# Aedelon/ProteinBERT-PyTorch-Replication

Measured on AMD Instinct MI355X. Metric: sequences/sec (whole node) ProteinBERT pretrain L=512 at 1/2/4/8 MI355X, higher is better.
Workload: dtype bf16; 1 GPU; global_batch=2048, per_gpu_batch=2048, seq_len=512, parallelism=dp1, impl=hip, hip_graph=False

## Files before the change

### proteinbert_pytorch_replication_amd/ops/csrc/common.h

```cpp
#pragma once
#include <hip/hip_runtime.h>
#include <stdint.h>

#define PBX_EXPORT extern "C" __attribute__((visibility("default")))

typedef __attribute__((ext_vector_type(8))) short bf16x8_t;
typedef __attribute__((ext_vector_type(4))) short bf16x4_t;
typedef __attribute__((ext_vector_type(4))) float f32x4_t;
typedef __attribute__((ext_vector_type(16))) float f32x16_t;

__device__ __forceinline__ float bf2f(unsigned short h) {
  return __uint_as_float(((unsigned int)h) << 16);
}
__device__ __forceinline__ unsigned short f2bf(float f) {
  return __builtin_bit_cast(unsigned short, (__bf16)f);
}

__device__ __forceinline__ void gelu_parts(float x, float& cdf, float& pdf) {
  const float z = fabsf(x) * 0.70710678118654752f;
  const float t = __builtin_amdgcn_rcpf(fmaf(0.3275911f, z, 1.0f));
  const float e = __expf(-z * z);
  const float poly =
      t * fmaf(t, fmaf(t, fmaf(t, fmaf(t, 1.061405429f, -1.453152027f), 1.421413741f), -0.284496736f), 0.254829592f);
  const float erfz = fmaf(-poly, e, 1.0f);
  cdf = fmaf(0.5f, copysignf(erfz, x), 0.5f);
  pdf = 0.3989422804014327f * e;
}
__device__ __forceinline__ float gelu_f(float x) {
  float c, p;
  gelu_parts(x, c, p);
  return x * c;
}
__device__ __forceinline__ float gelu_grad_f(float x) {
  float c, p;
  gelu_parts(x, c, p);
  return fmaf(x, p, c);
}

typedef float f32x2 __attribute__((ext_vector_type(2)));

#ifndef PBX_GELU_EXACT
#define PBX_GELU_EXACT 0
#endif

template <int N, int MODE>
__device__ __forceinline__ void gelu_scalar_n(const f32x2* x, f32x2* g, f32x2* gd) {
  constexpr int M = 2 * N;
  float xs[M], t[M], e[M], pl[M];
#pragma unroll
  for (int i = 0; i < M; ++i) {
    xs[i] = (i & 1) ? x[i >> 1].y : x[i >> 1].x;
    t[i] = fmaf(fabsf(xs[i]), 0.23164190f, 1.0f);
    e[i] = MODE == 0 ? (xs[i] * -0.72134752044448170f) * xs[i]
                     : fmaf(xs[i] * xs[i], -0.72134752044448170f, -1.3257480647361592f);
  }
#pragma unroll
  for (int i = 0; i < M; ++i) {
    t[i] = __builtin_amdgcn_rcpf(t[i]);
    e[i] = __builtin_amdgcn_exp2f(e[i]);
  }
  constexpr float c5 = MODE == 0 ? -0.5307027145f : -1.3302744295891233f;
  constexpr float c4 = MODE == 0 ? 0.7265760135f : 1.8212559791077754f;
  constexpr float c3 = MODE == 0 ? -0.7107068705f : -1.7814779365698128f;
  constexpr float c2 = MODE == 0 ? 0.142248368f : 0.3565637812489156f;
  constexpr float c1 = MODE == 0 ? -0.127414796f : -0.31938153025994087f;
#pragma unroll
  for (int i = 0; i < M; ++i) pl[i] = fmaf(t[i], c5, c4);
#pragma unroll
  for (int i = 0; i < M; ++i) pl[i] = fmaf(t[i], pl[i], c3);
#pragma unroll
  for (int i = 0; i < M; ++i) pl[i] = fmaf(t[i], pl[i], c2);
#pragma unroll
  for (int i = 0; i < M; ++i) pl[i] = fmaf(t[i], pl[i], c1);
#pragma unroll
  for (int i = 0; i < M; ++i) pl[i] = fmaf(pl[i] * t[i], e[i], 0.5f);
#pragma unroll
  for (int i = 0; i < M; ++i) {
    float gv = 0.f, dv = 0.f;
    if (MODE == 0) {
      gv = fmaf(fabsf(xs[i]), pl[i], xs[i] * 0.5f);
    } else {
      const float Phi = copysignf(pl[i], xs[i]) + 0.5f;
      if (MODE == 2) gv = xs[i] * Phi;
      dv = fmaf(xs[i], e[i], Phi);
    }
    if (i & 1) {
      if (MODE != 1) g[i >> 1].y = gv;
      if (MODE != 0) gd[i >> 1].y = dv;
    } else {
      if (MODE != 1) g[i >> 1].x = gv;
      if (MODE != 0) gd[i >> 1].x = dv;
    }
  }
}

template <int N, int MODE>
__device__ __forceinline__ void gelu_logistic_n(const f32x2* x, f32x2* g, f32x2* gd) {
  constexpr int M = 2 * N;
  float xs[M], t[M], s[M];
#pragma unroll
  for (int i = 0; i < M; ++i) {
    xs[i] = (i & 1) ? x[i >> 1].y : x[i >> 1].x;
    t[i] = xs[i] * xs[i];
    s[i] = fmaf(t[i], -0.10053117f, -2.3073633f) * xs[i];
  }
#pragma unroll
  for (int i = 0; i < M; ++i) s[i] = __builtin_amdgcn_rcpf(__builtin_amdgcn_exp2f(s[i]) + 1.0f);
#pragma unroll
  for (int i = 0; i < M; ++i) {
    float gv = 0.f, dv = 0.f;
    if (MODE != 1) gv = xs[i] * s[i];
    if (MODE != 0) {
      const float kd = fmaf(t[i], 0.20904868f, 1.59934236f);
      dv = fmaf(xs[i] * fmaf(-s[i], s[i], s[i]), kd, s[i]);
    }
    if (i & 1) {
      if (MODE != 1) g[i >> 1].y = gv;
      if (MODE != 0) gd[i >> 1].y = dv;
    } else {
      if (MODE != 1) g[i >> 1].x = gv;
      if (MODE != 0) gd[i >> 1].x = dv;
    }
  }
}

template <int N, int MODE>
__device__ __forceinline__ void gelu_n(const f32x2* x, f32x2* g, f32x2* gd) {
  if constexpr (PBX_GELU_EXACT) gelu_scalar_n<N, MODE>(x, g, gd);
  else gelu_logistic_n<N, MODE>(x, g, gd);
}
template <int N, bool GRAD>
__device__ __forceinline__ void gelu2_fast_n(const f32x2* x, f32x2* out) {
  if (GRAD) gelu_n<N, 1>(x, nullptr, out);
  else gelu_n<N, 0>(x, out, nullptr);
}
template <int N>
__device__ __forceinline__ void gelu2_both_n(const f32x2* x, f32x2* g, f32x2* gd) {
  gelu_n<N, 2>(x, g, gd);
}

__device__ __forceinline__ float wave_reduce_sum(float v) {
#pragma unroll
  for (int o = 32; o > 0; o >>= 1) v += __shfl_xor(v, o, 64);
  return v;
}
__device__ __forceinline__ float wave_reduce_max(float v) {
#pragma unroll
  for (int o = 32; o > 0; o >>= 1) v = fmaxf(v, __shfl_xor(v, o, 64));
  return v;
}

__device__ __forceinline__ unsigned long long pbx_mix64(unsigned long long z) {
  z += 0x9E3779B97F4A7C15ull;
  z = (z ^ (z >> 30)) * 0xBF58476D1CE4E5B9ull;
  z = (z ^ (z >> 27)) * 0x94D049BB133111EBull;
  return z ^ (z >> 31);
}
__device__ __forceinline__ float pbx_uniform(unsigned long long seed, unsigned long long stream,
                                             unsigned long long idx) {
  unsigned long long h = pbx_mix64(seed ^ pbx_mix64(stream * 0xD1B54A32D192ED03ull + idx));
  return (float)(h >> 40) * (1.0f / 16777216.0f);
}

static inline int pbx_launch_status() { return (int)hipGetLastError(); }
```

### proteinbert_pytorch_replication_amd/ops/csrc/ln.hip

```cpp
#include "mfma.h"
#include <stdlib.h>

using namespace pbx;
typedef unsigned short bf16_t;

namespace {
constexpr int CH = 128;
constexpr int BML = 32;

__device__ __forceinline__ void load_f8(const float* p, float* v) {
  const float4 a = *reinterpret_cast<const float4*>(p);
  const float4 c = *reinterpret_cast<const float4*>(p + 4);
  v[0] = a.x; v[1] = a.y; v[2] = a.z; v[3] = a.w; v[4] = c.x; v[5] = c.y; v[6] = c.z; v[7] = c.w;
}

__device__ __forceinline__ void stage_weight(unsigned char* dst, const bf16_t* __restrict__ w, int rows) {
  stage_chunks(
      rows * 16, [&](int idx) { return *reinterpret_cast<const uint4*>(w + (size_t)idx * 8); },
      [&](int idx, uint4 v) { *reinterpret_cast<uint4*>(dst + swz256(idx >> 4, idx & 15)) = v; });
}

constexpr int PB = 32;
constexpr int YS = CH + 4;

__device__ __forceinline__ uint4 ldq(const bf16_t* p, bool ok) {
  return ok ? *reinterpret_cast<const uint4*>(p) : make_uint4(0u, 0u, 0u, 0u);
}

__device__ __forceinline__ void sample_stats(float* sh, const float* __restrict__ st, int T, int BM, int L, float eps,
                                             const float* __restrict__ sums, int Ts, float inv_n) {
  if (threadIdx.x == 0) {
    float mean, rstd;
    ln_stats(st, T, BM, L, CH, eps, mean, rstd);
    sh[0] = mean;
    sh[1] = rstd;
    if (sums != nullptr) {
      float m1, m2;
      ln_bwd_consts(sums, Ts, inv_n, m1, m2);
      sh[2] = m1;
      sh[3] = m2;
    }
  }
}

__global__ void __launch_bounds__(512) ln_linear_fwd_kernel(
    const bf16_t* __restrict__ s1, const float* __restrict__ st1, int T1, int BM1, const float* __restrict__ g1,
    const float* __restrict__ be1, const bf16_t* __restrict__ wl, const float* __restrict__ bl,
    bf16_t* __restrict__ pre_l, bf16_t* __restrict__ s2, float* __restrict__ st2, int B, int L, float eps) {
  extern __shared__ __attribute__((aligned(16))) unsigned char smem[];
  unsigned char* ws = smem;
  unsigned char* ht = smem + 32768;
  float* yt = reinterpret_cast<float*>(smem + 32768 + PB * 256);
  float* tab = yt + PB * YS;
  const int tid = threadIdx.x, lane = tid & 63, w = tid >> 6;
  const int r = lane & 31, h = lane >> 5;
  const int j = tid >> 4, ch = tid & 15;
  const int l0 = blockIdx.x * PB, l = l0 + j;
  const bool okl = l < L;
  const int TP = (L + PB - 1) / PB;
  const int nbg = gridDim.y;
  const int b0 = (int)((long)B * blockIdx.y / nbg), b1 = (int)((long)B * (blockIdx.y + 1) / nbg);
  const int nb = b1 - b0;
  float* part = tab + 2 * nb;
  stage_weight(ws, wl, CH);
  for (int i = w; i < nb; i += 8) {
    float mean, rstd;
    wave_ln_stats(st1 + (size_t)(b0 + i) * T1 * 2, T1, BM1, L, CH, eps, mean, rstd);
    if (lane == 0) {
      tab[2 * i] = mean;
      tab[2 * i + 1] = rstd;
    }
  }
  float gam[8] = {0, 0, 0, 0, 0, 0, 0, 0}, bet[8] = {0, 0, 0, 0, 0, 0, 0, 0}, bb[8];
  if (okl) {
    load_f8(g1 + (size_t)l * CH + ch * 8, gam);
    load_f8(be1 + (size_t)l * CH + ch * 8, bet);
  }
  load_f8(bl + ch * 8, bb);
  uint4 nxt = ldq(s1 + ((size_t)b0 * L + l) * CH + ch * 8, okl && nb > 0);
  __syncthreads();
  for (int b = b0; b < b1; ++b) {
    const int i = b - b0;
    const float mean = tab[2 * i], rstd = tab[2 * i + 1];
    float sv[8], h1[8];
    unpack8(nxt, sv);
#pragma unroll
    for (int e = 0; e < 8; ++e) h1[e] = okl ? (sv[e] - mean) * rstd * gam[e] + bet[e] : 0.f;
    *reinterpret_cast<uint4*>(ht + swz256(j, ch)) = packq8(h1);
    __syncthreads();
    nxt = ldq(s1 + ((size_t)(b + 1) * L + l) * CH + ch * 8, okl && b + 1 < b1);
    if (w < 4) {
      f32x16_t acc = zero16();
#pragma unroll
      for (int kk = 0; kk < 8; ++kk)
        acc = mfma32(lds_frag(ws, swz256(w * 32 + r, kk * 2 + h)), lds_frag(ht, swz256(r, kk * 2 + h)), acc);
#pragma unroll
      for (int g = 0; g < 4; ++g)
        *reinterpret_cast<float4*>(yt + r * YS + w * 32 + 8 * g + 4 * h) =
            make_float4(acc[4 * g], acc[4 * g + 1], acc[4 * g + 2], acc[4 * g + 3]);
    }
    __syncthreads();
    float pre[8], o[8];
    const float4 ya = *reinterpret_cast<const float4*>(yt + j * YS + ch * 8);
    const float4 yb = *reinterpret_cast<const float4*>(yt + j * YS + ch * 8 + 4);
    const float yv[8] = {ya.x, ya.y, ya.z, ya.w, yb.x, yb.y, yb.z, yb.w};
#pragma unroll
    for (int e = 0; e < 8; ++e) pre[e] = yv[e] + bb[e];
    f32x2 gg[4];
    {
      const f32x2 xi[4] = {(f32x2){pre[0], pre[1]}, (f32x2){pre[2], pre[3]}, (f32x2){pre[4], pre[5]},
                           (f32x2){pre[6], pre[7]}};
      gelu2_fast_n<4, false>(xi, gg);
    }
#pragma unroll
    for (int e = 0; e < 8; ++e) o[e] = h1[e] + ((e & 1) ? gg[e >> 1].y : gg[e >> 1].x);
    const uint4 oq = packq8(o);
    if (okl) {
      const size_t off = ((size_t)b * L + l) * CH + ch * 8;
      if (pre_l != nullptr) *reinterpret_cast<uint4*>(pre_l + off) = packq8(pre);
      *reinterpret_cast<uint4*>(s2 + off) = oq;
    }
    float orr[8];
    unpack8(oq, orr);
    float sa = 0.f, sq = 0.f;
#pragma unroll
    for (int e = 0; e < 8; ++e) {
      sa += orr[e];
      sq += orr[e] * orr[e];
    }
    sa = wave_reduce_sum(okl ? sa : 0.f);
    sq = wave_reduce_sum(okl ? sq : 0.f);
    if (lane == 0) { part[(i * 8 + w) * 2] = sa; part[(i * 8 + w) * 2 + 1] = sq; }
  }
  __syncthreads();
  const int vrows = min(PB, L - l0);
  for (int i = tid; i < nb; i += 512) {
    float sa = 0.f, sq = 0.f;
#pragma unroll
    for (int ww = 0; ww < 8; ++ww) {
      sa += part[(i * 8 + ww) * 2];
      sq += part[(i * 8 + ww) * 2 + 1];
    }
    const float m = sa / (float)(vrows * CH);
    st2[((size_t)(b0 + i) * TP + blockIdx.x) * 2] = m;
    st2[((size_t)(b0 + i) * TP + blockIdx.x) * 2 + 1] = fmaxf(sq - sa * m, 0.f);
  }
}

__global__ void __launch_bounds__(256) ln2_consts_kernel(const float* __restrict__ st2, int T2, int BM2,
                                                         const float* __restrict__ sums2, int TS2,
                                                         const float* __restrict__ st1, int T1, int BM1,
                                                         float* __restrict__ consts, float* __restrict__ zero128,
                                                         int B, int L, float eps) {
  const int b = blockIdx.x * 4 + (threadIdx.x >> 6);
  if (b >= B) return;
  if (zero128 != nullptr)
    *reinterpret_cast<float2*>(zero128 + (size_t)b * CH + 2 * (threadIdx.x & 63)) = make_float2(0.f, 0.f);
  float mean2, rstd2, m1, m2, mean1, rstd1;
  wave_ln_stats(st2 + (size_t)b * T2 * 2, T2, BM2, L, CH, eps, mean2, rstd2);
  wave_bwd_consts(sums2 + (size_t)b * TS2 * 2, TS2, 1.0f / (float)(L * CH), m1, m2);
  wave_ln_stats(st1 + (size_t)b * T1 * 2, T1, BM1, L, CH, eps, mean1, rstd1);
  if ((threadIdx.x & 63) == 0) {
    float4* c = reinterpret_cast<float4*>(consts + (size_t)b * 8);
    c[0] = make_float4(mean2, rstd2, m1, m2);
    c[1] = make_float4(mean1, rstd1, 0.f, 0.f);
  }
}

__global__ void __launch_bounds__(512) ln2_linear_bwd_kernel(
    const bf16_t* __restrict__ dh2, const bf16_t* __restrict__ s2, const float* __restrict__ g2,
    const bf16_t* __restrict__ pre_l, const bf16_t* __restrict__ s1,
    const float* __restrict__ g1, const float* __restrict__ be1, const bf16_t* __restrict__ wl,
    const float* __restrict__ consts,
    bf16_t* __restrict__ dh1, float* __restrict__ sums1, float* __restrict__ dg2, float* __restrict__ db2,
    float* __restrict__ dg1, float* __restrict__ db1, float* __restrict__ dwl, float* __restrict__ dbl,
    float* __restrict__ dwl_slab, float* __restrict__ dbl_slab, int B, int L) {
  extern __shared__ __attribute__((aligned(16))) unsigned char smem[];
  unsigned char* ws = smem;
  unsigned char* dt = smem + 32768;
  unsigned char* ht = dt + 32 * 256;
  float* yt = reinterpret_cast<float*>(ht + 32 * 256);
  const int tid = threadIdx.x, lane = tid & 63, w = tid >> 6;
  const int r = lane & 31, h = lane >> 5;
  const int q = tr_q(lane), tc = tr_c(lane);
  const int j = tid >> 4, ch = tid & 15;
  const int TS1 = (L + 1) / 2;
  const int nsplit = gridDim.y;
  const int b0 = (int)((long)B * blockIdx.y / nsplit), b1 = (int)((long)B * (blockIdx.y + 1) / nsplit);
  stage_weight(ws, wl, CH);
  float adbl[8] = {0, 0, 0, 0, 0, 0, 0, 0};
  f32x16_t aw0 = zero16(), aw1 = zero16();
  const int wco = (w >> 1) * 32, wci = (w & 1) * 64;
  for (int pair = blockIdx.x; pair < TS1; pair += gridDim.x) {
    const int l = pair * 2 + (j & 1);
    const bool okl = l < L;
    float ga2[8] = {0, 0, 0, 0, 0, 0, 0, 0}, ga1[8] = {0, 0, 0, 0, 0, 0, 0, 0}, bt1[8] = {0, 0, 0, 0, 0, 0, 0, 0};
    if (okl) {
      load_f8(g2 + (size_t)l * CH + ch * 8, ga2);
      load_f8(g1 + (size_t)l * CH + ch * 8, ga1);
      load_f8(be1 + (size_t)l * CH + ch * 8, bt1);
    }
    float adg2[8] = {0, 0, 0, 0, 0, 0, 0, 0}, adb2[8] = {0, 0, 0, 0, 0, 0, 0, 0};
    float adg1[8] = {0, 0, 0, 0, 0, 0, 0, 0}, adb1[8] = {0, 0, 0, 0, 0, 0, 0, 0};
    const size_t coff = (size_t)l * CH + ch * 8;
    int bs = b0 + (j >> 1);
    bool ok = okl && bs < b1;
    size_t off = (size_t)bs * L * CH + coff;
    uint4 n_dh = ldq(dh2 + off, ok), n_s2 = ldq(s2 + off, ok), n_s1 = ldq(s1 + off, ok);
    uint4 n_pr = ldq(pre_l + off, ok);
    float4 n_c0 = make_float4(0.f, 1.f, 0.f, 0.f), n_c1 = make_float4(0.f, 1.f, 0.f, 0.f);
    if (bs < b1) {
      n_c0 = *reinterpret_cast<const float4*>(consts + (size_t)bs * 8);
      n_c1 = *reinterpret_cast<const float4*>(consts + (size_t)bs * 8 + 4);
    }
    for (int bc = b0; bc < b1; bc += 16) {
      const int bcur = bs;
      const bool okc = ok;
      const size_t offc = off;
      const float mean2 = n_c0.x, rstd2 = n_c0.y, m1 = n_c0.z, m2 = n_c0.w, mean1 = n_c1.x, rstd1 = n_c1.y;
      float dh[8], sv2[8], pr[8], sv1[8], ds2[8], dp[8], xh1[8], hv[8];
      unpack8(n_dh, dh);
      unpack8(n_s2, sv2);
      unpack8(n_s1, sv1);
#pragma unroll
      for (int e = 0; e < 8; ++e) {
        const float xh2 = (sv2[e] - mean2) * rstd2;
        adg2[e] += okc ? dh[e] * xh2 : 0.f;
        adb2[e] += okc ? dh[e] : 0.f;
        ds2[e] = okc ? rstd2 * (dh[e] * ga2[e] - m1 - xh2 * m2) : 0.f;
        xh1[e] = (sv1[e] - mean1) * rstd1;
        hv[e] = okc ? xh1[e] * ga1[e] + bt1[e] : 0.f;
      }
      *reinterpret_cast<uint4*>(ht + swz256(j, ch)) = packq8(hv);
      auto prefetch = [&]() {
        bs = bc + 16 + (j >> 1);
        ok = okl && bs < b1;
        off = (size_t)bs * L * CH + coff;
        n_dh = ldq(dh2 + off, ok);
        n_s2 = ldq(s2 + off, ok);
        n_pr = ldq(pre_l + off, ok);
        n_s1 = ldq(s1 + off, ok);
        if (bs < b1) {
          n_c0 = *reinterpret_cast<const float4*>(consts + (size_t)bs * 8);
          n_c1 = *reinterpret_cast<const float4*>(consts + (size_t)bs * 8 + 4);
        }
      };
      unpack8(n_pr, pr);
      float gp[8];
      {
        const f32x2 xi[4] = {(f32x2){pr[0], pr[1]}, (f32x2){pr[2], pr[3]}, (f32x2){pr[4], pr[5]},
                             (f32x2){pr[6], pr[7]}};
        f32x2 go[4];
        gelu2_fast_n<4, true>(xi, go);
#pragma unroll
        for (int e = 0; e < 4; ++e) {
          gp[2 * e] = go[e].x;
          gp[2 * e + 1] = go[e].y;
        }
      }
#pragma unroll
      for (int e = 0; e < 8; ++e) dp[e] = ds2[e] * gp[e];
      const uint4 dq = packq8(dp);
      *reinterpret_cast<uint4*>(dt + swz256(j, ch)) = dq;
      {
        float dpr[8];
        unpack8(dq, dpr);
#pragma unroll
        for (int e = 0; e < 8; ++e) adbl[e] += dpr[e];
      }
      __syncthreads();
      prefetch();
      if (w < 4) {
        f32x16_t acc = zero16();
#pragma unroll
        for (int kk = 0; kk < 8; ++kk) {
          const int rlo = kk * 16 + 8 * h + q;
          const int col = w * 32 + tc;
          const bf16x8 fa = cat_tr(lds_tr(ws, swz256e(rlo, col)), lds_tr(ws, swz256e(rlo + 4, col)));
          acc = mfma32(fa, lds_frag(dt, swz256(r, kk * 2 + h)), acc);
        }
#pragma unroll
        for (int g = 0; g < 4; ++g)
          *reinterpret_cast<float4*>(yt + r * YS + w * 32 + 8 * g + 4 * h) =
              make_float4(acc[4 * g], acc[4 * g + 1], acc[4 * g + 2], acc[4 * g + 3]);
      }
#pragma unroll
      for (int ks = 0; ks < 2; ++ks) {
        const int rlo = ks * 16 + 8 * h + q;
        const bf16x8 fa = cat_tr(lds_tr(dt, swz256e(rlo, wco + tc)), lds_tr(dt, swz256e(rlo + 4, wco + tc)));
        const bf16x8 fb0 = cat_tr(lds_tr(ht, swz256e(rlo, wci + tc)), lds_tr(ht, swz256e(rlo + 4, wci + tc)));
        const bf16x8 fb1 =
            cat_tr(lds_tr(ht, swz256e(rlo, wci + 32 + tc)), lds_tr(ht, swz256e(rlo + 4, wci + 32 + tc)));
        aw0 = mfma32(fa, fb0, aw0);
        aw1 = mfma32(fa, fb1, aw1);
      }
      __syncthreads();
      const float4 ya = *reinterpret_cast<const float4*>(yt + j * YS + ch * 8);
      const float4 yb = *reinterpret_cast<const float4*>(yt + j * YS + ch * 8 + 4);
      const float yv[8] = {ya.x, ya.y, ya.z, ya.w, yb.x, yb.y, yb.z, yb.w};
      float o[8], sa = 0.f, sc = 0.f;
#pragma unroll
      for (int e = 0; e < 8; ++e) {
        o[e] = okc ? bfround(ds2[e] + yv[e]) : 0.f;
        const float dxh = o[e] * ga1[e];
        sa += dxh;
        sc += dxh * xh1[e];
        adg1[e] += o[e] * xh1[e];
        adb1[e] += o[e];
      }
      if (okc) *reinterpret_cast<uint4*>(dh1 + offc) = packq8(o);
#pragma unroll
      for (int m = 1; m <= 16; m <<= 1) {
        sa += __shfl_xor(sa, m, 64);
        sc += __shfl_xor(sc, m, 64);
      }
      if ((lane & 31) == 0 && bcur < b1) {
        sums1[((size_t)bcur * TS1 + pair) * 2] = sa;
        sums1[((size_t)bcur * TS1 + pair) * 2 + 1] = sc;
      }
    }
    const int l0 = pair * 2;
    float* accs[4] = {adg2, adb2, adg1, adb1};
    float* dsts[4] = {dg2, db2, dg1, db1};
#pragma unroll
    for (int a = 0; a < 4; ++a) {
      __syncthreads();
#pragma unroll
      for (int e = 0; e < 8; ++e) yt[j * CH + ch * 8 + e] = accs[a][e];
      __syncthreads();
      if (tid < 2 * CH) {
        const int par = tid >> 7, c = tid & (CH - 1);
        float v = 0.f;
#pragma unroll
        for (int k = 0; k < 16; ++k) v += yt[(2 * k + par) * CH + c];
        if (l0 + par < L) atomicAdd(dsts[a] + (size_t)(l0 + par) * CH + c, v);
      }
    }
    __syncthreads();
  }
  __syncthreads();
#pragma unroll
  for (int e = 0; e < 8; ++e) yt[j * CH + ch * 8 + e] = adbl[e];
  __syncthreads();
  if (tid < CH) {
    float a = 0.f;
#pragma unroll 8
    for (int k = 0; k < 32; ++k) a += yt[k * CH + tid];
    if (dbl_slab != nullptr) dbl_slab[(size_t)(blockIdx.y * gridDim.x + blockIdx.x) * CH + tid] = a;
    else atomicAdd(dbl + tid, a);
  }
  float* dw = dwl_slab != nullptr ? dwl_slab + (size_t)(blockIdx.y * gridDim.x + blockIdx.x) * CH * CH : dwl;
#pragma unroll
  for (int i = 0; i < 16; ++i) {
    const int co = wco + (i & 3) + 8 * (i >> 2) + 4 * h;
    if (dwl_slab != nullptr) {
      dw[(size_t)co * CH + wci + r] = aw0[i];
      dw[(size_t)co * CH + wci + 32 + r] = aw1[i];
    } else {
      atomicAdd(dw + (size_t)co * CH + wci + r, aw0[i]);
      atomicAdd(dw + (size_t)co * CH + wci + 32 + r, aw1[i]);
    }
  }
}

__global__ void __launch_bounds__(512) ln1_finalize_kernel(
    const bf16_t* __restrict__ dh1, const bf16_t* __restrict__ s1, const float* __restrict__ st1, int T1, int BM1,
    const float* __restrict__ sums1, int TS1, const float* __restrict__ g1, bf16_t* __restrict__ ds1,
    float* __restrict__ dgb, int B, int L, float eps) {
  extern __shared__ __attribute__((aligned(16))) unsigned char smem[];
  float* red = reinterpret_cast<float*>(smem);
  float* tab = red + 2 * PB * CH;
  const int tid = threadIdx.x, lane = tid & 63, w = tid >> 6;
  const int j = tid >> 4, ch = tid & 15;
  const int nbg = gridDim.y;
  const int b0 = (int)((long)B * blockIdx.y / nbg), b1 = (int)((long)B * (blockIdx.y + 1) / nbg);
  const int nb = b1 - b0;
  float* dacc = tab + 4 * nb;
  const float inv_n = 1.0f / (float)(L * CH);
  for (int i = w; i < nb; i += 8) {
    float mean, rstd, m1, m2;
    wave_ln_stats(st1 + (size_t)(b0 + i) * T1 * 2, T1, BM1, L, CH, eps, mean, rstd);
    wave_bwd_consts(sums1 + (size_t)(b0 + i) * TS1 * 2, TS1, inv_n, m1, m2);
    if (lane == 0) { tab[4 * i] = mean; tab[4 * i + 1] = rstd; tab[4 * i + 2] = m1; tab[4 * i + 3] = m2; }
  }
  for (int i = tid; i < nb * CH; i += 512) dacc[i] = 0.f;
  const int TP = (L + PB - 1) / PB;
  int it = 0;
  for (int px = blockIdx.x; px < TP; px += gridDim.x) {
    const int l = px * PB + j;
    const bool okl = l < L;
    float ga[8] = {0, 0, 0, 0, 0, 0, 0, 0};
    if (okl) load_f8(g1 + (size_t)l * CH + ch * 8, ga);
    const size_t coff = (size_t)min(l, L - 1) * CH + ch * 8;
    uint4 n_dh = *reinterpret_cast<const uint4*>(dh1 + (size_t)min(b0, B - 1) * L * CH + coff);
    uint4 n_s = *reinterpret_cast<const uint4*>(s1 + (size_t)min(b0, B - 1) * L * CH + coff);
    __syncthreads();
    for (int b = b0; b < b1; ++b, ++it) {
      const float* tb = tab + 4 * (b - b0);
      const float mean = tb[0], rstd = tb[1], m1 = tb[2], m2 = tb[3];
      float* rb = red + (it & 1) * PB * CH;
      float dv[8], sv[8], o[8];
      unpack8(n_dh, dv);
      unpack8(n_s, sv);
      const size_t noff = (size_t)min(b + 1, B - 1) * L * CH + coff;
      n_dh = *reinterpret_cast<const uint4*>(dh1 + noff);
      n_s = *reinterpret_cast<const uint4*>(s1 + noff);
#pragma unroll
      for (int e = 0; e < 8; ++e) o[e] = okl ? rstd * (dv[e] * ga[e] - m1 - (sv[e] - mean) * rstd * m2) : 0.f;
      const uint4 qv = packq8(o);
      if (okl) *reinterpret_cast<uint4*>(ds1 + (size_t)b * L * CH + (size_t)l * CH + ch * 8) = qv;
      unpack8(qv, o);
#pragma unroll
      for (int e = 0; e < 8; ++e) {
        o[e] += __shfl_xor(o[e], 16, 64);
        o[e] += __shfl_xor(o[e], 32, 64);
      }
      if (lane < 16) {
        *reinterpret_cast<float4*>(rb + w * CH + ch * 8) = make_float4(o[0], o[1], o[2], o[3]);
        *reinterpret_cast<float4*>(rb + w * CH + ch * 8 + 4) = make_float4(o[4], o[5], o[6], o[7]);
      }
      __syncthreads();
      if (tid < CH) {
        float a = 0.f;
#pragma unroll
        for (int k = 0; k < 8; ++k) a += rb[k * CH + tid];
        dacc[(b - b0) * CH + tid] += a;
      }
    }
  }
  __syncthreads();
  for (int i = tid; i < nb * CH; i += 512) atomicAdd(dgb + (size_t)(b0 + i / CH) * CH + i % CH, dacc[i]);
}

__global__ void __launch_bounds__(256) embed_fwd_kernel(const long long* __restrict__ tok, const float* __restrict__ E,
                                                        bf16_t* __restrict__ out, long rows) {
  const long i = (long)blockIdx.x * 256 + threadIdx.x;
  if (i >= rows * 16) return;
  const long row = i >> 4;
  const int c8 = (int)(i & 15);
  const long long t = tok[row];
  float v[8];
  load_f8(E + (size_t)t * CH + c8 * 8, v);
  *reinterpret_cast<uint4*>(out + row * CH + c8 * 8) = packq8(v);
}

template <bool DPRE>
__global__ void __launch_bounds__(256) embed_bwd_kernel(const long long* __restrict__ tok,
                                                        const bf16_t* __restrict__ dout, float* __restrict__ dE,
                                                        long rows, int V, float* __restrict__ slab,
                                                        const bf16_t* __restrict__ gdn, const bf16_t* __restrict__ gdw,
                                                        bf16_t* __restrict__ dpn, bf16_t* __restrict__ dpw) {
  __shared__ __attribute__((aligned(16))) unsigned char ds[256 * 256];
  __shared__ int ts[256];
  const int tid = threadIdx.x, lane = tid & 63, w = tid >> 6;
  const int r = lane & 31, h = lane >> 5;
  const int q = tr_q(lane), tc = tr_c(lane);
  const long per = (rows + gridDim.x - 1) / gridDim.x;
  const long r0 = (long)blockIdx.x * per, r1 = min(rows, r0 + per);
  f32x16_t acc = zero16();
  for (long t0 = r0; t0 < r1; t0 += 256) {
    const int n = (int)min((long)256, r1 - t0);
    __syncthreads();
    if constexpr (DPRE) {
      for (int base = tid; base < 256 * 16; base += 4 * 256) {
        uint4 gq[4], nq[4], wq[4];
#pragma unroll
        for (int i = 0; i < 4; ++i) {
          const int idx = base + i * 256, row = idx >> 4;
          const size_t off = (size_t)(t0 + min(row, n - 1)) * CH + (idx & 15) * 8;
          gq[i] = *reinterpret_cast<const uint4*>(dout + off);
          nq[i] = *reinterpret_cast<const uint4*>(gdn + off);
          wq[i] = *reinterpret_cast<const uint4*>(gdw + off);
        }
#pragma unroll
        for (int i = 0; i < 4; ++i) {
          const int idx = base + i * 256, row = idx >> 4;
          const bool ok = row < n;
          *reinterpret_cast<uint4*>(ds + swz256(row, idx & 15)) = ok ? gq[i] : make_uint4(0u, 0u, 0u, 0u);
          if (ok) {
            float g[8], pn[8], pw[8], on[8], ow[8];
            unpack8(gq[i], g);
            unpack8(nq[i], pn);
            unpack8(wq[i], pw);
#pragma unroll
            for (int e = 0; e < 8; ++e) {
              on[e] = pn[e] * g[e];
              ow[e] = pw[e] * g[e];
            }
            const size_t off = (size_t)(t0 + row) * CH + (idx & 15) * 8;
            *reinterpret_cast<uint4*>(dpn + off) = packq8(on);
            *reinterpret_cast<uint4*>(dpw + off) = packq8(ow);
          }
        }
      }
    } else {
      stage_chunks(
          256 * 16,
          [&](int idx) {
            const int row = idx >> 4;
            return row < n ? *reinterpret_cast<const uint4*>(dout + (t0 + row) * CH + (idx & 15) * 8)
                           : make_uint4(0u, 0u, 0u, 0u);
          },
          [&](int idx, uint4 v) { *reinterpret_cast<uint4*>(ds + swz256(idx >> 4, idx & 15)) = v; });
    }
    ts[tid] = tid < n ? (int)tok[t0 + tid] : -1;
    __syncthreads();
    const int colb = w * 32 + tc;
#pragma unroll 4
    for (int kb = 0; kb < 16; ++kb) {
      typedef __attribute__((ext_vector_type(8))) unsigned short u16x8;
      u16x8 oh;
#pragma unroll
      for (int j = 0; j < 8; ++j) oh[j] = ts[kb * 16 + 8 * h + j] == r ? (unsigned short)0x3F80 : (unsigned short)0;
      const int rb = kb * 16 + 8 * h + q;
      const bf16x8 fb = cat_tr(lds_tr(ds, swz256e(rb, colb)), lds_tr(ds, swz256e(rb + 4, colb)));
      acc = mfma32(__builtin_bit_cast(bf16x8, oh), fb, acc);
    }
  }
#pragma unroll
  for (int i = 0; i < 16; ++i) {
    const int v = (i & 3) + 8 * (i >> 2) + 4 * h;
    if (slab != nullptr) {
      if (v < V) slab[((size_t)blockIdx.x * V + v) * CH + w * 32 + r] = acc[i];
    } else if (v < V && acc[i] != 0.f) {
      atomicAdd(dE + v * CH + w * 32 + r, acc[i]);
    }
  }
}

int g_cus = -1;
int num_cus() {
  if (g_cus < 0) {
    int dev = 0;
    g_cus = 256;
    if (hipGetDevice(&dev) == hipSuccess) {
      hipDeviceProp_t p;
      if (hipGetDeviceProperties(&p, dev) == hipSuccess) g_cus = p.multiProcessorCount;
    }
  }
  return g_cus;
}
int persistent_grid(int tiles, int per_cu) {
  const int cap = num_cus() * per_cu;
  return tiles < cap ? (tiles > 0 ? tiles : 1) : cap;
}
}

extern "C" int pbx_colsum_add(const float* src, int rows, int cols, float* dst, const float* scale, hipStream_t st);

static bool ln_attrs_set = false;
static void set_ln_attrs() {
  if (ln_attrs_set) return;
  (void)hipFuncSetAttribute((const void*)ln_linear_fwd_kernel, hipFuncAttributeMaxDynamicSharedMemorySize, 163840);
  (void)hipFuncSetAttribute((const void*)ln2_linear_bwd_kernel, hipFuncAttributeMaxDynamicSharedMemorySize, 163840);
  (void)hipFuncSetAttribute((const void*)ln1_finalize_kernel, hipFuncAttributeMaxDynamicSharedMemorySize, 163840);
  ln_attrs_set = true;
}

static int ln_groups(int B, int L) {
  const int tp = (L + PB - 1) / PB;
  int g = (2 * num_cus() + tp - 1) / tp;
  return g < 1 ? 1 : (g > B ? B : g);
}

PBX_EXPORT int pbx_ln_linear_fwd(const void* s1, const float* st1, int T1, int BM1, const float* g1,
                                 const float* be1, const void* wl, const float* bl, void* pre_l, void* s2,
                                 float* st2, int B, int L, float eps, hipStream_t st) {
  dim3 grid((L + PB - 1) / PB, ln_groups(B, L));
  const int nbmax = (B + (int)grid.y - 1) / (int)grid.y;
  const int lds = 32768 + PB * 256 + PB * YS * 4 + nbmax * 18 * 4;
  if (lds > 163840) return (int)hipErrorInvalidValue;
  set_ln_attrs();
  hipLaunchKernelGGL(ln_linear_fwd_kernel, grid, dim3(512), lds, st, (const bf16_t*)s1, st1, T1, BM1, g1, be1,
                     (const bf16_t*)wl, bl, (bf16_t*)pre_l, (bf16_t*)s2, st2, B, L, eps);
  return pbx_launch_status();
}

static void ln2_bwd_grid(int B, int L, int det, int& gx, int& nsplit) {
  const int pairs = (L + 1) / 2;
  const int target = num_cus();
  nsplit = (target + pairs - 1) / pairs;
  if (nsplit > (B + 15) / 16) nsplit = (B + 15) / 16;
  if (nsplit < 1 || det) nsplit = 1;
  gx = pairs < target ? pairs : target;
}

PBX_EXPORT int pbx_ln2_bwd_slab_rows(int B, int L, int det) {
  int gx, nsplit;
  ln2_bwd_grid(B, L, det, gx, nsplit);
  return gx * nsplit;
}

PBX_EXPORT int pbx_ln2_linear_bwd(const void* dh2, const void* s2, const float* st2, const float* sums2, int TS2,
                                  const float* g2, const void* pre_l, const void* s1, const float* st1, int T1,
                                  int BM1, const float* g1, const float* be1, const void* wl, float* consts,
                                  void* dh1, float* sums1, float* dg2, float* db2, float* dg1, float* db1, float* dwl,
                                  float* dbl, float* dgb_zero, int B, int L, float eps, float* dwl_slab, int slab_rows,
                                  int det, int fold, int consts_ready, hipStream_t st) {
  set_ln_attrs();
  const int T2 = (L + PB - 1) / PB;
  if (!consts_ready)
    hipLaunchKernelGGL(ln2_consts_kernel, dim3((B + 3) / 4), dim3(256), 0, st, st2, T2, PB, sums2, TS2, st1, T1, BM1,
                       consts, dgb_zero, B, L, eps);
  int gx, nsplit;
  ln2_bwd_grid(B, L, det, gx, nsplit);
  const int lds = 32768 + 2 * 32 * 256 + 32 * YS * 4;
  const int nwg = gx * nsplit;
  float* slab = dwl_slab != nullptr && nwg <= slab_rows ? dwl_slab : nullptr;
  float* bslab = slab != nullptr ? slab + (size_t)slab_rows * CH * CH : nullptr;
  if ((det || !fold) && slab == nullptr) return (int)hipErrorInvalidValue;
  hipLaunchKernelGGL(ln2_linear_bwd_kernel, dim3(gx, nsplit), dim3(512), lds, st, (const bf16_t*)dh2,
                     (const bf16_t*)s2, g2, (const bf16_t*)pre_l, (const bf16_t*)s1, g1, be1, (const bf16_t*)wl,
                     consts, (bf16_t*)dh1, sums1, dg2, db2, dg1, db1, dwl, dbl, slab, bslab, B, L);
  if (slab != nullptr && fold) {
    int rc = pbx_launch_status();
    if (rc != 0) return rc;
    rc = pbx_colsum_add(slab, nwg, CH * CH, dwl, nullptr, st);
    if (rc != 0) return rc;
    return pbx_colsum_add(bslab, nwg, CH, dbl, nullptr, st);
  }
  return pbx_launch_status();
}

PBX_EXPORT int pbx_ln1_finalize(const void* dh1, const void* s1, const float* st1, int T1, int BM1,
                                const float* sums1, int TS1, const float* g1, void* ds1, float* dgb, int B, int L,
                                float eps, int det, hipStream_t st) {
  const int tp = (L + PB - 1) / PB;
  const int gx = det ? 1 : (tp < 16 ? tp : 16);
  int gy = (2 * num_cus() + gx - 1) / gx;
  gy = gy < 1 ? 1 : (gy > B ? B : gy);
  dim3 grid(gx, gy);
  const int nbmax = (B + (int)grid.y - 1) / (int)grid.y;
  const int lds = 2 * PB * CH * 4 + nbmax * 16 + nbmax * CH * 4;
  if (lds > 163840) return (int)hipErrorInvalidValue;
  set_ln_attrs();
  hipLaunchKernelGGL(ln1_finalize_kernel, grid, dim3(512), lds, st, (const bf16_t*)dh1, (const bf16_t*)s1, st1, T1,
                     BM1, sums1, TS1, g1, (bf16_t*)ds1, dgb, B, L, eps);
  return pbx_launch_status();
}

PBX_EXPORT int pbx_embed_fwd(const void* tok, const float* E, void* out, long rows, hipStream_t st) {
  const long n = rows * 16;
  hipLaunchKernelGGL(embed_fwd_kernel, dim3((unsigned)((n + 255) / 256)), dim3(256), 0, st, (const long long*)tok, E,
                     (bf16_t*)out, rows);
  return pbx_launch_status();
}

PBX_EXPORT int pbx_embed_bwd_groups(long rows) {
  long g = (rows + 511) / 512;
  if (g > 2 * num_cus()) g = 2 * num_cus();
  return g < 1 ? 1 : (int)g;
}

PBX_EXPORT int pbx_embed_bwd(const void* tok, const void* dout, float* dE, long rows, int V, float* slab,
                             hipStream_t st) {
  if (V > 32) return (int)hipErrorInvalidValue;
  const int g = pbx_embed_bwd_groups(rows);
  hipLaunchKernelGGL(embed_bwd_kernel<false>, dim3((unsigned)g), dim3(256), 0, st, (const long long*)tok,
                     (const bf16_t*)dout, dE, rows, V, slab, nullptr, nullptr, nullptr, nullptr);
  if (slab != nullptr) {
    const int rc = pbx_launch_status();
    if (rc != 0) return rc;
    return pbx_colsum_add(slab, g, V * CH, dE, nullptr, st);
  }
  return pbx_launch_status();
}

PBX_EXPORT int pbx_embed_dpre(const void* tok, const void* ds1, const void* gdn, const void* gdw, void* dpn, void* dpw,
                              float* dE, long rows, int V, float* slab, hipStream_t st) {
  if (V > 32 || rows < 1) return (int)hipErrorInvalidValue;
  const int g = pbx_embed_bwd_groups(rows);
  hipLaunchKernelGGL(embed_bwd_kernel<true>, dim3((unsigned)g), dim3(256), 0, st, (const long long*)tok,
                     (const bf16_t*)ds1, dE, rows, V, slab, (const bf16_t*)gdn, (const bf16_t*)gdw, (bf16_t*)dpn,
                     (bf16_t*)dpw);
  if (slab != nullptr) {
    const int rc = pbx_launch_status();
    if (rc != 0) return rc;
    return pbx_colsum_add(slab, g, V * CH, dE, nullptr, st);
  }
  return pbx_launch_status();
}
```

### proteinbert_pytorch_replication_amd/ops/csrc/mfma.h

```cpp
#pragma once
#include "common.h"

typedef __attribute__((ext_vector_type(8))) __bf16 bf16x8;
typedef __attribute__((ext_vector_type(4))) short s16x4;

namespace pbx {

__device__ __forceinline__ f32x16_t mfma32(const bf16x8& a, const bf16x8& b, const f32x16_t& c) {
  return __builtin_amdgcn_mfma_f32_32x32x16_bf16(a, b, c, 0, 0, 0);
}

__device__ __forceinline__ f32x16_t zero16() {
  f32x16_t z;
#pragma unroll
  for (int i = 0; i < 16; ++i) z[i] = 0.f;
  return z;
}

__device__ __forceinline__ int swz256(int row, int chunk) {
  return (row << 8) + ((chunk ^ (((row & 3) << 2) | ((row >> 2) & 3))) << 4);
}
__device__ __forceinline__ int swz256e(int row, int col) {
  return swz256(row, col >> 3) + ((col & 7) << 1);
}
__device__ __forceinline__ int swz128(int row, int chunk) {
  return (row << 7) + ((chunk ^ ((row >> 1) & 7)) << 4);
}

__device__ __forceinline__ bf16x8 lds_frag(const unsigned char* base, int byte_off) {
  return *reinterpret_cast<const bf16x8*>(base + byte_off);
}

__device__ __forceinline__ s16x4 lds_tr(const unsigned char* base, int byte_off) {
  typedef __attribute__((address_space(3))) s16x4 lds_s16x4;
  return __builtin_amdgcn_ds_read_tr16_b64_v4i16((lds_s16x4*)(base + byte_off));
}

__device__ __forceinline__ bf16x8 cat_tr(const s16x4& lo, const s16x4& hi) {
  typedef __attribute__((ext_vector_type(8))) short s16x8;
  s16x8 v;
  v[0] = lo[0]; v[1] = lo[1]; v[2] = lo[2]; v[3] = lo[3];
  v[4] = hi[0]; v[5] = hi[1]; v[6] = hi[2]; v[7] = hi[3];
  return __builtin_bit_cast(bf16x8, v);
}

__device__ __forceinline__ int tr_q(int lane) { return (lane >> 2) & 3; }
__device__ __forceinline__ int tr_c(int lane) { return ((lane & 3) << 2) + (((lane >> 4) & 1) << 4); }

__device__ __forceinline__ bf16x8 pack8(const float* v) {
  typedef __attribute__((ext_vector_type(8))) unsigned short u16x8;
  u16x8 u;
#pragma unroll
  for (int i = 0; i < 8; ++i) u[i] = f2bf(v[i]);
  return __builtin_bit_cast(bf16x8, u);
}

__device__ __forceinline__ void unpack8(const uint4& q, float* v) {
  v[0] = __uint_as_float(q.x << 16); v[1] = __uint_as_float(q.x & 0xffff0000u);
  v[2] = __uint_as_float(q.y << 16); v[3] = __uint_as_float(q.y & 0xffff0000u);
  v[4] = __uint_as_float(q.z << 16); v[5] = __uint_as_float(q.z & 0xffff0000u);
  v[6] = __uint_as_float(q.w << 16); v[7] = __uint_as_float(q.w & 0xffff0000u);
}
__device__ __forceinline__ void unpack4(const uint2& q, float* v) {
  v[0] = __uint_as_float(q.x << 16); v[1] = __uint_as_float(q.x & 0xffff0000u);
  v[2] = __uint_as_float(q.y << 16); v[3] = __uint_as_float(q.y & 0xffff0000u);
}
__device__ __forceinline__ uint4 packq8(const float* v) {
  uint4 q;
  q.x = (unsigned)f2bf(v[0]) | ((unsigned)f2bf(v[1]) << 16);
  q.y = (unsigned)f2bf(v[2]) | ((unsigned)f2bf(v[3]) << 16);
  q.z = (unsigned)f2bf(v[4]) | ((unsigned)f2bf(v[5]) << 16);
  q.w = (unsigned)f2bf(v[6]) | ((unsigned)f2bf(v[7]) << 16);
  return q;
}
__device__ __forceinline__ uint2 packq4(const float* v) {
  uint2 q;
  q.x = (unsigned)f2bf(v[0]) | ((unsigned)f2bf(v[1]) << 16);
  q.y = (unsigned)f2bf(v[2]) | ((unsigned)f2bf(v[3]) << 16);
  return q;
}
__device__ __forceinline__ float bfround(float f) { return bf2f(f2bf(f)); }

__device__ __forceinline__ float block_sum(float v, float* scratch, int nw) {
  v = wave_reduce_sum(v);
  const int w = threadIdx.x >> 6;
  __syncthreads();
  if ((threadIdx.x & 63) == 0) scratch[w] = v;
  __syncthreads();
  float s = 0.f;
  for (int i = 0; i < nw; ++i) s += scratch[i];
  return s;
}

__device__ __forceinline__ void ln_stats(const float* __restrict__ part, int T, int BM, int L, int C, float eps,
                                         float& mean, float& rstd) {
  float n = 0.f, m = 0.f, M2 = 0.f;
  for (int t = 0; t < T; ++t) {
    const float nt = (float)(min(BM, L - t * BM) * C);
    const float mt = part[2 * t], M2t = part[2 * t + 1];
    const float nn = n + nt;
    const float d = mt - m;
    m += d * (nt / nn);
    M2 += M2t + d * d * (n * nt / nn);
    n = nn;
  }
  mean = m;
  rstd = rsqrtf(M2 / n + eps);
}

__device__ __forceinline__ void ln_bwd_consts(const float* __restrict__ part, int T, float inv_n, float& m1,
                                              float& m2) {
  float a = 0.f, c = 0.f;
  for (int t = 0; t < T; ++t) { a += part[2 * t]; c += part[2 * t + 1]; }
  m1 = a * inv_n;
  m2 = c * inv_n;
}

template <typename SrcF, typename DstF>
__device__ __forceinline__ void stage_chunks(int n, SrcF src, DstF dst) {
  const int bs = blockDim.x;
  for (int base = threadIdx.x; base < n; base += 8 * bs) {
    uint4 v[8];
#pragma unroll
    for (int i = 0; i < 8; ++i) {
      const int idx = base + i * bs;
      v[i] = idx < n ? src(idx) : make_uint4(0u, 0u, 0u, 0u);
    }
#pragma unroll
    for (int i = 0; i < 8; ++i) {
      const int idx = base + i * bs;
      if (idx < n) dst(idx, v[i]);
    }
  }
}

__device__ __forceinline__ void chan_merge(float& n, float& m, float& M2, float nb, float mb, float M2b) {
  const float nn = n + nb;
  if (nn > 0.f) {
    const float d = mb - m;
    const float f = nb / nn;
    m += d * f;
    M2 += M2b + d * d * n * f;
  }
  n = nn;
}

__device__ __forceinline__ void wave_ln_stats(const float* __restrict__ part, int T, int BM, int L, int C, float eps,
                                              float& mean, float& rstd) {
  const int lane = threadIdx.x & 63;
  float n = 0.f, m = 0.f, M2 = 0.f;
  for (int t = lane; t < T; t += 64) {
    const float2 pm = *reinterpret_cast<const float2*>(part + 2 * t);
    chan_merge(n, m, M2, (float)(min(BM, L - t * BM) * C), pm.x, pm.y);
  }
#pragma unroll
  for (int o = 32; o >= 1; o >>= 1) {
    const float nb = __shfl_xor(n, o, 64), mb = __shfl_xor(m, o, 64), M2b = __shfl_xor(M2, o, 64);
    chan_merge(n, m, M2, nb, mb, M2b);
  }
  mean = m;
  rstd = rsqrtf(M2 / n + eps);
}

__device__ __forceinline__ void wave_bwd_consts(const float* __restrict__ part, int T, float inv_n, float& m1,
                                                float& m2) {
  const int lane = threadIdx.x & 63;
  float a = 0.f, c = 0.f;
  for (int t = lane; t < T; t += 64) {
    const float2 pm = *reinterpret_cast<const float2*>(part + 2 * t);
    a += pm.x;
    c += pm.y;
  }
  m1 = wave_reduce_sum(a) * inv_n;
  m2 = wave_reduce_sum(c) * inv_n;
}

__device__ __forceinline__ void wave_chan(float& n, float& m, float& M2) {
#pragma unroll
  for (int o = 32; o >= 1; o >>= 1) {
    const float nb = __shfl_xor(n, o, 64), mb = __shfl_xor(m, o, 64), M2b = __shfl_xor(M2, o, 64);
    chan_merge(n, m, M2, nb, mb, M2b);
  }
}

}
```

Baseline: 109,700 sequences/s.

## Use buffer loads/stores with range-checked descriptors in LN backward, pack bf16 pairs

Rewrites the LN-linear backward inner loop so global loads and stores go through AMD buffer resources whose size bounds replace per-element branches. Out-of-range lanes get a drop offset, and dummy dropped stores plus compiler barriers are inserted to shape issue order. It also adds a paired float-to-bf16 conversion used by the pack helpers, and rounds the output once via packq8/unpack8. The aim is fewer branches and address computations and cheaper conversions, at the cost of fragile inline-asm ordering tricks and extra dummy stores.

```diff
diff --git a/proteinbert_pytorch_replication_amd/ops/csrc/common.h b/proteinbert_pytorch_replication_amd/ops/csrc/common.h
--- a/proteinbert_pytorch_replication_amd/ops/csrc/common.h
+++ b/proteinbert_pytorch_replication_amd/ops/csrc/common.h
@@ -38,6 +38,11 @@
 }
 
 typedef float f32x2 __attribute__((ext_vector_type(2)));
+
+__device__ __forceinline__ unsigned f2bf2(float a, float b) {
+  typedef __bf16 bf16x2_t __attribute__((ext_vector_type(2)));
+  return __builtin_bit_cast(unsigned, __builtin_convertvector((f32x2){a, b}, bf16x2_t));
+}
 
 #ifndef PBX_GELU_EXACT
 #define PBX_GELU_EXACT 0
diff --git a/proteinbert_pytorch_replication_amd/ops/csrc/ln.hip b/proteinbert_pytorch_replication_amd/ops/csrc/ln.hip
--- a/proteinbert_pytorch_replication_amd/ops/csrc/ln.hip
+++ b/proteinbert_pytorch_replication_amd/ops/csrc/ln.hip
@@ -26,6 +26,44 @@
 __device__ __forceinline__ uint4 ldq(const bf16_t* p, bool ok) {
   return ok ? *reinterpret_cast<const uint4*>(p) : make_uint4(0u, 0u, 0u, 0u);
 }
+
+typedef __attribute__((ext_vector_type(4))) unsigned int u32x4;
+typedef __attribute__((ext_vector_type(2))) unsigned int u32x2;
+constexpr int VO_DROP = 0x7ffffff0;
+__device__ __forceinline__ __amdgpu_buffer_rsrc_t buf_rsrc(const void* base, int bytes) {
+  return __builtin_amdgcn_make_buffer_rsrc(const_cast<void*>(base), (short)0, bytes, 0x00020000);
+}
+__device__ __forceinline__ uint4 ldq(const __amdgpu_buffer_rsrc_t& rs, int vo) {
+  const u32x4 v = __builtin_amdgcn_raw_buffer_load_b128(rs, vo, 0, 0);
+  return make_uint4(v[0], v[1], v[2], v[3]);
+}
+__device__ __forceinline__ void stq(const __amdgpu_buffer_rsrc_t& rs, int vo, const uint4& q) {
+  __builtin_amdgcn_raw_buffer_store_b128((u32x4){q.x, q.y, q.z, q.w}, rs, vo, 0, 0);
+}
+
+template <int N>
+__device__ __forceinline__ void retire(const float* v) {
+#pragma unroll
+  for (int e = 0; e < N; ++e) asm volatile("" ::"v"(v[e]));
+}
+__device__ __forceinline__ void issue_fence() { asm volatile("" ::: "memory"); }
+template <class T>
+__device__ __forceinline__ const T* opaque(const T* p) {
+  asm volatile("" : "+s"(p));
+  return p;
+}
+template <int N>
+__device__ __forceinline__ void dropped_stores(void* base) {
+  const __amdgpu_buffer_rsrc_t none = buf_rsrc(base, 0);
+  issue_fence();
+#pragma unroll
+  for (int i = 0; i < N; ++i) {
+    __builtin_amdgcn_raw_buffer_store_b32(0u, none, VO_DROP - 16 * i, 0, 0);
+    issue_fence();
+  }
+}
+
+constexpr int FWD_RING = 1;
 
 __device__ __forceinline__ void sample_stats(float* sh, const float* __restrict__ st, int T, int BM, int L, float eps,
                                              const float* __restrict__ sums, int Ts, float inv_n) {
@@ -188,40 +226,66 @@
   const int nsplit = gridDim.y;
   const int b0 = (int)((long)B * blockIdx.y / nsplit), b1 = (int)((long)B * (blockIdx.y + 1) / nsplit);
   stage_weight(ws, wl, CH);
+  const bf16_t *const dh2o = opaque(dh2), *const s2o = opaque(s2), *const pre_lo = opaque(pre_l), *const s1o = opaque(s1);
+  const float* const constso = opaque(consts);
   float adbl[8] = {0, 0, 0, 0, 0, 0, 0, 0};
   f32x16_t aw0 = zero16(), aw1 = zero16();
   const int wco = (w >> 1) * 32, wci = (w & 1) * 64;
   for (int pair = blockIdx.x; pair < TS1; pair += gridDim.x) {
     const int l = pair * 2 + (j & 1);
     const bool okl = l < L;
-    float ga2[8] = {0, 0, 0, 0, 0, 0, 0, 0}, ga1[8] = {0, 0, 0, 0, 0, 0, 0, 0}, bt1[8] = {0, 0, 0, 0, 0, 0, 0, 0};
-    if (okl) {
-      load_f8(g2 + (size_t)l * CH + ch * 8, ga2);
-      load_f8(g1 + (size_t)l * CH + ch * 8, ga1);
-      load_f8(be1 + (size_t)l * CH + ch * 8, bt1);
-    }
+    const int coff = min(l, L - 1) * CH + ch * 8;
+    float ga2[8], ga1[8], bt1[8];
+    load_f8(g2 + coff, ga2);
+    load_f8(g1 + coff, ga1);
+    load_f8(be1 + coff, bt1);
+#pragma unroll
+    for (int e = 0; e < 8; ++e) {
+      ga2[e] = okl ? ga2[e] : 0.f;
+      ga1[e] = okl ? ga1[e] : 0.f;
+      bt1[e] = okl ? bt1[e] : 0.f;
+    }
+    retire<8>(ga2);
+    retire<8>(ga1);
+    retire<8>(bt1);
     float adg2[8] = {0, 0, 0, 0, 0, 0, 0, 0}, adb2[8] = {0, 0, 0, 0, 0, 0, 0, 0};
     float adg1[8] = {0, 0, 0, 0, 0, 0, 0, 0}, adb1[8] = {0, 0, 0, 0, 0, 0, 0, 0};
-    const size_t coff = (size_t)l * CH + ch * 8;
-    int bs = b0 + (j >> 1);
-    bool ok = okl && bs < b1;
-    size_t off = (size_t)bs * L * CH + coff;
-    uint4 n_dh = ldq(dh2 + off, ok), n_s2 = ldq(s2 + off, ok), n_s1 = ldq(s1 + off, ok);
-    uint4 n_pr = ldq(pre_l + off, ok);
-    float4 n_c0 = make_float4(0.f, 1.f, 0.f, 0.f), n_c1 = make_float4(0.f, 1.f, 0.f, 0.f);
-    if (bs < b1) {
-      n_c0 = *reinterpret_cast<const float4*>(consts + (size_t)bs * 8);
-      n_c1 = *reinterpret_cast<const float4*>(consts + (size_t)bs * 8 + 4);
-    }
+    const int blast = max(b1 - 1, 0);
+    const int vo_dh = okl ? (((j >> 1) * L + l) * CH + ch * 8) * 2 : VO_DROP;
+    const int vo_su = (lane & 31) == 0 ? ((j >> 1) * TS1 + pair) * 8 : VO_DROP;
+    bool ok, okb;
+    uint4 n_dh, n_s2, n_pr, n_s1;
+    float4 n_c0, n_c1;
+    auto prefetch = [&](int bc) {
+      const int bs = bc + (j >> 1);
+      okb = bs < b1;
+      ok = okl && okb;
+      const int cb = min(bc, blast), ns = min(b1 - cb, 16);
+      const int sm = min(bs, blast) - cb;
+      const int vl = (sm * L * CH + coff) * 2, bytes = ns * L * CH * 2;
+      const size_t base = (size_t)cb * L * CH;
+      n_dh = ldq(buf_rsrc(dh2o + base, bytes), vl);
+      n_s2 = ldq(buf_rsrc(s2o + base, bytes), vl);
+      n_pr = ldq(buf_rsrc(pre_lo + base, bytes), vl);
+      n_s1 = ldq(buf_rsrc(s1o + base, bytes), vl);
+      const __amdgpu_buffer_rsrc_t rc = buf_rsrc(constso + (size_t)cb * 8, ns * 32);
+      const uint4 q0 = ldq(rc, sm * 32), q1 = ldq(rc, sm * 32 + 16);
+      n_c0 = make_float4(__uint_as_float(q0.x), __uint_as_float(q0.y), __uint_as_float(q0.z), __uint_as_float(q0.w));
+      n_c1 = make_float4(__uint_as_float(q1.x), __uint_as_float(q1.y), __uint_as_float(q1.z), __uint_as_float(q1.w));
+    };
+    issue_fence();
+    prefetch(b0);
+    dropped_stores<2>(dh1);
     for (int bc = b0; bc < b1; bc += 16) {
-      const int bcur = bs;
       const bool okc = ok;
-      const size_t offc = off;
-      const float mean2 = n_c0.x, rstd2 = n_c0.y, m1 = n_c0.z, m2 = n_c0.w, mean1 = n_c1.x, rstd1 = n_c1.y;
+      const uint4 zq = make_uint4(0u, 0u, 0u, 0u);
+      const float4 c0 = okb ? n_c0 : make_float4(0.f, 1.f, 0.f, 0.f);
+      const float4 c1 = okb ? n_c1 : make_float4(0.f, 1.f, 0.f, 0.f);
+      const float mean2 = c0.x, rstd2 = c0.y, m1 = c0.z, m2 = c0.w, mean1 = c1.x, rstd1 = c1.y;
       float dh[8], sv2[8], pr[8], sv1[8], ds2[8], dp[8], xh1[8], hv[8];
-      unpack8(n_dh, dh);
-      unpack8(n_s2, sv2);
-      unpack8(n_s1, sv1);
+      unpack8(okc ? n_dh : zq, dh);
+      unpack8(okc ? n_s2 : zq, sv2);
+      unpack8(okc ? n_s1 : zq, sv1);
 #pragma unroll
       for (int e = 0; e < 8; ++e) {
         const float xh2 = (sv2[e] - mean2) * rstd2;
@@ -232,20 +296,7 @@
         hv[e] = okc ? xh1[e] * ga1[e] + bt1[e] : 0.f;
       }
       *reinterpret_cast<uint4*>(ht + swz256(j, ch)) = packq8(hv);
-      auto prefetch = [&]() {
-        bs = bc + 16 + (j >> 1);
-        ok = okl && bs < b1;
-        off = (size_t)bs * L * CH + coff;
-        n_dh = ldq(dh2 + off, ok);
-        n_s2 = ldq(s2 + off, ok);
-        n_pr = ldq(pre_l + off, ok);
-        n_s1 = ldq(s1 + off, ok);
-        if (bs < b1) {
-          n_c0 = *reinterpret_cast<const float4*>(consts + (size_t)bs * 8);
-          n_c1 = *reinterpret_cast<const float4*>(consts + (size_t)bs * 8 + 4);
-        }
-      };
-      unpack8(n_pr, pr);
+      unpack8(okc ? n_pr : zq, pr);
       float gp[8];
       {
         const f32x2 xi[4] = {(f32x2){pr[0], pr[1]}, (f32x2){pr[2], pr[3]}, (f32x2){pr[4], pr[5]},
@@ -269,7 +320,7 @@
         for (int e = 0; e < 8; ++e) adbl[e] += dpr[e];
       }
       __syncthreads();
-      prefetch();
+      prefetch(bc + 16);
       if (w < 4) {
         f32x16_t acc = zero16();
 #pragma unroll
@@ -300,24 +351,26 @@
       const float yv[8] = {ya.x, ya.y, ya.z, ya.w, yb.x, yb.y, yb.z, yb.w};
       float o[8], sa = 0.f, sc = 0.f;
 #pragma unroll
+      for (int e = 0; e < 8; ++e) o[e] = okc ? ds2[e] + yv[e] : 0.f;
+      const uint4 oq = packq8(o);
+      unpack8(oq, o);
+#pragma unroll
       for (int e = 0; e < 8; ++e) {
-        o[e] = okc ? bfround(ds2[e] + yv[e]) : 0.f;
         const float dxh = o[e] * ga1[e];
         sa += dxh;
         sc += dxh * xh1[e];
         adg1[e] += o[e] * xh1[e];
         adb1[e] += o[e];
       }
-      if (okc) *reinterpret_cast<uint4*>(dh1 + offc) = packq8(o);
+      const int nsmp = min(b1 - bc, 16);
+      stq(buf_rsrc(dh1 + (size_t)bc * L * CH, nsmp * L * CH * 2), vo_dh, oq);
 #pragma unroll
       for (int m = 1; m <= 16; m <<= 1) {
         sa += __shfl_xor(sa, m, 64);
         sc += __shfl_xor(sc, m, 64);
       }
-      if ((lane & 31) == 0 && bcur < b1) {
-        sums1[((size_t)bcur * TS1 + pair) * 2] = sa;
-        sums1[((size_t)bcur * TS1 + pair) * 2 + 1] = sc;
-      }
+      __builtin_amdgcn_raw_buffer_store_b64((u32x2){__float_as_uint(sa), __float_as_uint(sc)},
+                                            buf_rsrc(sums1 + (size_t)bc * TS1 * 2, nsmp * TS1 * 8), vo_su, 0, 0);
     }
     const int l0 = pair * 2;
     float* accs[4] = {adg2, adb2, adg1, adb1};
@@ -562,6 +615,8 @@
   int g = (2 * num_cus() + tp - 1) / tp;
   return g < 1 ? 1 : (g > B ? B : g);
 }
+
+PBX_EXPORT int pbx_ln_fwd_ring(void) { return FWD_RING; }
 
 PBX_EXPORT int pbx_ln_linear_fwd(const void* s1, const float* st1, int T1, int BM1, const float* g1,
                                  const float* be1, const void* wl, const float* bl, void* pre_l, void* s2,
diff --git a/proteinbert_pytorch_replication_amd/ops/csrc/mfma.h b/proteinbert_pytorch_replication_amd/ops/csrc/mfma.h
--- a/proteinbert_pytorch_replication_amd/ops/csrc/mfma.h
+++ b/proteinbert_pytorch_replication_amd/ops/csrc/mfma.h
@@ -48,10 +48,10 @@
 __device__ __forceinline__ int tr_c(int lane) { return ((lane & 3) << 2) + (((lane >> 4) & 1) << 4); }
 
 __device__ __forceinline__ bf16x8 pack8(const float* v) {
-  typedef __attribute__((ext_vector_type(8))) unsigned short u16x8;
-  u16x8 u;
+  typedef __attribute__((ext_vector_type(4))) unsigned int u32x4_t;
+  u32x4_t u;
 #pragma unroll
-  for (int i = 0; i < 8; ++i) u[i] = f2bf(v[i]);
+  for (int i = 0; i < 4; ++i) u[i] = f2bf2(v[2 * i], v[2 * i + 1]);
   return __builtin_bit_cast(bf16x8, u);
 }
 
@@ -67,16 +67,16 @@
 }
 __device__ __forceinline__ uint4 packq8(const float* v) {
   uint4 q;
-  q.x = (unsigned)f2bf(v[0]) | ((unsigned)f2bf(v[1]) << 16);
-  q.y = (unsigned)f2bf(v[2]) | ((unsigned)f2bf(v[3]) << 16);
-  q.z = (unsigned)f2bf(v[4]) | ((unsigned)f2bf(v[5]) << 16);
-  q.w = (unsigned)f2bf(v[6]) | ((unsigned)f2bf(v[7]) << 16);
+  q.x = f2bf2(v[0], v[1]);
+  q.y = f2bf2(v[2], v[3]);
+  q.z = f2bf2(v[4], v[5]);
+  q.w = f2bf2(v[6], v[7]);
   return q;
 }
 __device__ __forceinline__ uint2 packq4(const float* v) {
   uint2 q;
-  q.x = (unsigned)f2bf(v[0]) | ((unsigned)f2bf(v[1]) << 16);
-  q.y = (unsigned)f2bf(v[2]) | ((unsigned)f2bf(v[3]) << 16);
+  q.x = f2bf2(v[0], v[1]);
+  q.y = f2bf2(v[2], v[3]);
   return q;
 }
 __device__ __forceinline__ float bfround(float f) { return bf2f(f2bf(f)); }
```

Result: faster. 112,400 sequences/s, median of 6 (+2.4%).
